# wtaylor17/ImageCFGen-Pytorch

Hardware: AMD Instinct MI355X
Metric: ALI training images/sec (E+G+D step), MorphoMNIST bs=512/GPU (higher is better)
Workload: dtype f32; 1 GPU; image_scms/mnist.py ALI iteration (EG step + 2 D steps + diagnostics), MorphoMNIST 28x28x1 synthetic, bs=512/GPU, fp32 MFMA, mode=stepper+hipgraph; global_batch=512, parallelism=dp1

## Files before the change

### imagecfgen-pytorch_amd/ali_hip/_lib.py

```python
import ctypes
import os
from ctypes import POINTER, Structure, c_char_p, c_double, c_float, c_int32, c_int64, c_size_t, c_uint64, c_void_p

_HERE = os.path.dirname(os.path.abspath(__file__))
LIB_PATH = os.path.join(_HERE, "libali_hip.so")


class AliHipUnavailable(RuntimeError):
    pass


class AliConvGeom(Structure):
    _fields_ = [(n, c_int32) for n in ("B", "H", "W", "C", "P", "Q", "K", "R", "S", "stride", "pad")]


class AliEpilogue(Structure):
    _fields_ = [("bias", c_void_p), ("act", c_int32), ("slope", c_float), ("mask", c_void_p), ("mask_ld", c_int32),
                ("dact_y", c_void_p), ("dact", c_int32), ("dslope", c_float),
                ("bn_part", c_void_p), ("bn_mode", c_int32), ("bn_groups", c_int32), ("bn_stat_mask", c_void_p),
                ("bn_mask_ld", c_int32), ("bn_x", c_void_p), ("bn_mean", c_void_p), ("bn_invstd", c_void_p),
                ("bn_mask_in", c_void_p), ("bn_mask_pre", c_void_p), ("mfma_f16", c_int32),
                ("in16", c_void_p), ("w16", c_void_p), ("out16", c_void_p),
                ("tile_order", c_void_p), ("tile_order_n", c_int32), ("in_ld", c_int32), ("out_ld", c_int32),
                ("in_ch_live", c_int32), ("bn_slots", c_int32), ("dact_y16", c_void_p)]
# ... 59 lines not shown
    "ali_act_bwd": (c_int32, [c_void_p, c_void_p, c_void_p, c_int64, c_int32, c_float, c_void_p]),
    "ali_colsum": (c_int32, [c_void_p, c_int64, c_int32, c_int32, c_void_p, c_void_p, c_size_t, c_void_p]),
    "ali_rowmask_mul": (c_int32, [c_void_p, c_void_p, c_void_p, c_int32, c_int32, c_int32, c_void_p]),
    "ali_dropout_mask": (c_int32, [c_uint64, c_uint64, c_void_p, c_float, c_void_p, c_int64, c_void_p]),
    "ali_dropout_mask_multi": (c_int32, [c_uint64, c_void_p, POINTER(c_int64), POINTER(c_float), POINTER(c_int32),
                                         POINTER(c_int32), c_int32, c_void_p, c_void_p]),
    "ali_normal_fill": (c_int32, [c_uint64, c_void_p, c_uint64, c_void_p, c_int64, c_void_p]),
    "ali_batch_gather": (c_int32, [c_void_p, c_int32, c_void_p, c_int32, c_void_p, c_void_p, c_void_p, c_int64, c_int32,
                                   c_int32, c_int32, c_int32, c_void_p, c_void_p, c_void_p, c_void_p, c_void_p]),
    "ali_bn_stats": (c_int32, [c_void_p, c_void_p, c_int32, c_int32, c_int32, c_void_p, c_void_p, c_void_p, c_void_p,
                               c_float, c_float, c_int32, c_void_p, c_void_p, c_void_p, c_void_p, c_int32, c_int64,
                               c_void_p, c_size_t, c_void_p]),
    "ali_bn_apply": (c_int32, [c_void_p, c_void_p, c_void_p, c_void_p, c_void_p, c_void_p, c_int32, c_int32, c_int32,
                               c_int32, c_int64, c_void_p]),
    "ali_bn_bwd": (c_int32, [c_void_p, c_void_p, c_void_p, c_void_p, c_void_p, c_void_p, c_void_p, c_int32, c_int32,
                             c_int32, c_int32, c_float, c_void_p, c_void_p, c_void_p, c_void_p, c_size_t, c_void_p]),
    "ali_bn_stats_from_partials": (c_int32, [c_void_p, c_int32, c_int32, c_int32, c_int64, c_void_p, c_void_p, c_void_p,
                                             c_void_p, c_float, c_float, c_void_p, c_void_p, c_void_p, c_void_p, c_int64,
                                             c_void_p]),
    "ali_bn_bwd_from_partials": (c_int32, [c_void_p, c_int32, c_void_p, c_void_p, c_void_p, c_void_p, c_void_p, c_void_p,
                                           c_void_p, c_int32, c_int32, c_int32, c_int32, c_float, c_void_p, c_void_p,
                                           c_void_p, c_void_p]),
    "ali_ew_plan": (c_int32, [c_int32, c_int64, c_int32, c_int32, c_int32, c_int32, c_int32, POINTER(c_int32)]),
    "ali_bce_logits": (c_int32, [c_void_p, c_int32, c_float, c_float, c_void_p, c_void_p, c_void_p]),
    "ali_softmax_xent": (c_int32, [c_void_p, c_void_p, c_int32, c_int32, c_float, c_void_p, c_void_p, c_void_p,
                                  c_void_p, c_void_p, c_size_t, c_void_p]),
    "ali_vae_latent_fwd": (c_int32, [c_void_p, c_void_p, c_int32, c_void_p, c_void_p, c_uint64, c_void_p, c_uint64,
                                    c_int32, c_int32, c_int32, c_float, POINTER(c_void_p), POINTER(c_int32),
                                    POINTER(c_int32), POINTER(c_void_p), c_int32, c_void_p, c_int32, c_int32, c_int32,
                                    c_void_p, c_void_p, c_void_p, c_size_t, c_void_p]),
    "ali_vae_loglik": (c_int32, [c_void_p, c_void_p, c_int32, c_int32, c_int32, c_float, c_void_p, c_float, c_float,
                                c_void_p, c_void_p, c_void_p, c_size_t, c_void_p]),
    "ali_vae_latent_bwd": (c_int32, [c_void_p, c_int32, c_void_p, c_void_p, c_void_p, c_int32, c_int32, c_int32, c_int32,
                                    c_float, c_float, c_void_p, c_void_p, c_void_p, c_int32, c_int32, c_void_p, c_void_p]),
    "ali_row_dist": (c_int32, [c_void_p, c_int32, c_void_p, c_int32, c_int64, c_int32, c_void_p, c_void_p, c_size_t,
                              c_void_p]),
    "ali_cf_hinge": (c_int32, [c_void_p, c_void_p, c_void_p, c_void_p, c_float, c_int32, c_int32, c_void_p, c_void_p,
                              c_void_p]),
    "ali_cf_join": (c_int32, [c_void_p, c_int32, c_void_p, c_void_p, c_int32, c_int32, c_int64, c_void_p, c_void_p]),
    "ali_cf_input_fwd": (c_int32, [c_void_p, c_int32, c_void_p, c_int32, POINTER(AliCfSegment), c_int32,
                                  POINTER(c_void_p), c_int32, c_int32, c_int32, c_int32, c_void_p, c_void_p, c_int32,
                                  c_void_p]),
    "ali_cf_input_step": (c_int32, [c_void_p, c_int32, c_void_p, c_void_p, c_int32, POINTER(AliCfSegment), c_int32,
                                   POINTER(c_void_p), c_int32, c_int32, c_void_p, c_void_p, c_void_p, c_int32, c_int32,
                                   c_void_p, c_double, c_double, c_double, c_double, c_void_p, c_void_p]),
    "ali_cf_select": (c_int32, [c_void_p, c_void_p, c_void_p, c_int32, c_int32, c_void_p, c_void_p, c_void_p,
# ... 138 lines not shown
```

### imagecfgen-pytorch_amd/ali_hip/chain.py

```python
import weakref
from collections import namedtuple
from typing import List, Optional

import torch
import torch.nn as nn

from . import dropout as _dropout
from . import ops
from .ops import ACT_LEAKY, ACT_NONE, ACT_TANH


def _pad4(c: int) -> int:
    return (c + 3) // 4 * 4


class Stage:
    __slots__ = ("kind", "mod", "act", "slope", "pre", "pattern", "has_drop", "drop_p", "bn", "unflat", "index", "hw")

    def __init__(self, kind, mod, pre, index):
        self.kind, self.mod, self.pre, self.index = kind, mod, pre, index
        self.act, self.slope, self.unflat = ACT_NONE, 0.0, None
        self.hw = None
        self.pattern = [k for k, _ in pre]
        self.has_drop = "drop" in self.pattern
# ... 495 lines not shown
        yield
    return (yield from gen)


def chain_forward(*args, **kwargs):
    return drive(chain_forward_gen(*args, **kwargs))


def chain_backward(*args, **kwargs):
    return drive(chain_backward_gen(*args, **kwargs))


def _pre_ops(st: Stage, sv, bn_part, mask_applied: bool, groups: int):
    cur, mask, bn = sv.x_in, sv.mask, st.bn
    B, H, W, Cp = sv.in_shape
    rows = H * W
    sv.bn_stats = None
    if bn is None:
        return ops.rowmask_mul(cur, mask, B, rows, Cp) if (mask is not None and not mask_applied) else cur
    mask_in = mask if st.pattern == ["drop", "bn"] else None
    mask_post = mask if st.pattern == ["bn", "drop"] else None
    use_batch = sv.training or bn.running_mean is None
    momentum = bn.momentum
    if bn_part is not None:
        stg = ops.bn_stats_from_partials(bn_part[0], bn_part[1], groups, Cp, (B // groups) * rows, bn.weight.detach(),
                                         bn.bias.detach(), bn.running_mean, bn.running_var, momentum, bn.eps)
    else:
        stg = ops.bn_stats(cur, mask_in, B, rows, Cp, bn.weight.detach(), bn.bias.detach(), bn.running_mean,
                           bn.running_var, momentum, bn.eps, use_batch, groups=groups)
    if use_batch and bn.num_batches_tracked is not None:
        for _ in range(groups):
            _count_batch(bn)
    sv.bn_stats = stg if groups == 1 else [stg[gi] for gi in range(groups)]
    return ops.bn_apply(cur, stg, mask_in, mask_post, B, rows, Cp, groups=groups)


def _for_next_stage(nxt: Stage, sv, groups: int, lane):
    B, P, Q, K = sv.out_shape
    draw = lambda: _dropout.next_mask(B, K, nxt.drop_p, sv.x_in.device, K, lane=lane)
    if sv.training and nxt.pattern == ["drop"] and sv.route.fold_ok:
        return draw(), None, None
    early = bn_fwd = None
    if nxt.bn is not None and sv.route.bn_leave and (sv.training or nxt.bn.running_mean is None):
        if sv.training and nxt.pattern == ["drop", "bn"]:
            early = draw()
        slots, tile_rows, pixel_major = ops.conv_mtiles(sv.geom, 0)
        rows_g = (B // groups) * (1 if pixel_major else P * Q)
        if slots > 0 and (groups == 1 or (B % groups == 0 and rows_g % tile_rows == 0
                                          and (not pixel_major or B % tile_rows == 0))):
            part = torch.empty(2 * K * slots, dtype=torch.float32, device=sv.x_in.device)
            bn_fwd = (part, groups, early, slots)
    return None, early, bn_fwd


def _launch_fwd(plan: ChainPlan, st: Stage, sv, folded, bn_fwd, out_ld: int, jmask, alloc):
    t, y, m, c_log = sv.t, sv.y, st.mod, sv.c_log
    B, H, W, Cp = sv.in_shape
# ... 178 lines not shown
        slots = ops.conv_mtiles(g, 0 if rt.dgrad == "convT" else 1)[0] if rt.bn_reduce else 0
        if slots > 0:
            bn_red = (torch.empty(2 * Cp * slots, dtype=torch.float32, device=g_pre.device), slots)
            ep = ops.epilogue(bn_bwd=(bn_red[0], sv.x_in, sv.bn_stats[0], sv.bn_stats[1], mask_in, mask_pre, slots))
        else:
            ep = ops.epilogue()
    if rt.dgrad == "tconv1" and bn is None and sv.mask is None:
        ops.tconv1_dgrad(g_pre, 1, plan.packed(st, "fwd", Cp), dact_y, pact, pslope, gt, B, H, W, Cp, m.kernel_size[0],
                         m.kernel_size[1], m.padding[0])
    elif st.kind == "convT":
        ops.conv_fwd(g, g_pre, plan.packed(st, "dgrad", Cp), gt, ep, live=(None, sv.c_log))
        yield
    else:
        wc = H * W * Cp if rt.dgrad == "flat_gemm" else Cp
        ops.conv_bwd_data(g, g_pre, plan.packed(st, "dgrad", wc), gt, ep, in_ld=ld,
                          live=(wc if rt.dgrad == "flat_gemm" else sv.c_log, None))
        yield
    if bn is None:
        return gt
    use_batch = sv.training or bn.running_mean is None
    slope = pslope if pact == ACT_LEAKY else -1.0
    out = dict(want_gx=want, out_dgamma=grad_dst.get(id(bn.weight)) if need_params else None,
               out_dbeta=grad_dst.get(id(bn.bias)) if need_params else None)
    if bn_red is not None:
        dgam, dbet, gprev = ops.bn_bwd_from_partials(bn_red[0], bn_red[1], sv.x_in, gt, mask_in, mask_pre, sv.bn_stats,
                                                     bn.weight.detach(), B, H * W, Cp, use_batch, slope, **out)
    else:
        dgam, dbet, gprev = ops.bn_bwd(sv.x_in, gt, mask_in, mask_pre, sv.bn_stats, bn.weight.detach(), B, H * W, Cp,
                                       use_batch, slope, **out)
    if need_params:
        grads[id(bn.weight)], grads[id(bn.bias)] = dgam, dbet
    if pact == ACT_TANH and gprev is not None:
        gprev = ops.act_bwd(gprev, sv.x_in, ACT_TANH, 0.0)
    return gprev


def chain_backward_gen(plan: ChainPlan, saved, gy: torch.Tensor, c_log_in: int, need_gx: bool, need_params: bool = True,
                       grad_dst=None, gx_planes=None, gy_ld: int = 0, gy_pre: bool = False, in_act=None, fold=None):
    grads = {}
    grad_dst = grad_dst or {}
    n = len(plan.stages)
    last = plan.stages[-1]
    assert saved[0].c_log == c_log_in, "chain_backward: c_log_in differs from the forward pass's"
    if gy_ld:
        if not (gy_pre or last.act == ACT_NONE) or not join_ok(plan):
            raise ValueError("chain_backward(gy_ld=...): needs join_ok(plan) and a pre-activation gradient")
        g_pre = gy
# ... 165 lines not shown
```

### imagecfgen-pytorch_amd/ali_hip/ops.py

```python
import collections
import ctypes
from ctypes import byref, c_void_p

import numpy as np
import torch

from . import _lib
from ._lib import ACT_LEAKY, ACT_NONE, ACT_TANH, AliConvGeom, AliEpilogue

_WS = {}
_WS_BYTES = 256 << 20


def set_workspace_bytes(n: int):
    global _WS_BYTES
    _WS_BYTES = int(n)
    _WS.clear()


def workspace(device, slot: int = 0) -> torch.Tensor:
    key = (device.type, device.index if device.index is not None else torch.cuda.current_device(), slot)
    ws = _WS.get(key)
    if ws is None or ws.numel() < _WS_BYTES:
        ws = torch.zeros(_WS_BYTES, dtype=torch.uint8, device=device)
# ... 813 lines not shown
    _lib.check(lib.ali_bn_stats_from_partials(_chk(part, "part"), slots, groups, C, count, _opt(gamma), _opt(beta),
                                              _opt(running_mean), _opt(running_var), momentum, eps,
                                              c_void_p(st[0, 0].data_ptr()), c_void_p(st[0, 1].data_ptr()),
                                              c_void_p(st[0, 2].data_ptr()), c_void_p(st[0, 3].data_ptr()), 4 * C,
                                              _stream()), "ali_bn_stats_from_partials")
    return st[0] if groups == 1 else st


def bn_bwd_from_partials(part, slots, x, g, mask_in, mask_pre, st, gamma, B, rows_per_img, C, batch_stats, slope,
                         want_gx=True, out_dgamma=None, out_dbeta=None):
    lib = _lib.load()
    if out_dgamma is None or out_dbeta is None:
        dg = torch.empty(2, C, dtype=torch.float32, device=x.device)
        out_dgamma, out_dbeta = dg[0], dg[1]
    gx = torch.empty_like(x) if want_gx else None
    _lib.check(lib.ali_bn_bwd_from_partials(_chk(part, "part"), slots, _chk(x, "x"), _chk(g, "g"), _opt(mask_in),
                                            _opt(mask_pre), c_void_p(st[0].data_ptr()), c_void_p(st[1].data_ptr()),
                                            _opt(gamma), B, rows_per_img, C, int(batch_stats), float(slope),
                                            _chk(out_dgamma, "dgamma"), _chk(out_dbeta, "dbeta"), _opt(gx), _stream()),
               "ali_bn_bwd_from_partials")
    return out_dgamma, out_dbeta, gx


def bn_apply(x, st, mask_in, mask_post, B, rows_per_img, C, out=None, groups=1):
    lib = _lib.load()
    out = torch.empty_like(x) if out is None else out
    st0 = st if groups == 1 else st[0]
    _lib.check(lib.ali_bn_apply(_chk(x, "x"), c_void_p(st0[2].data_ptr()), c_void_p(st0[3].data_ptr()), _opt(mask_in),
                                _opt(mask_post), _chk(out), B, rows_per_img, C, groups, 4 * C, _stream()),
               "ali_bn_apply")
    return out


def bn_bwd(x, g, mask_in, mask_pre, st, gamma, B, rows_per_img, C, batch_stats, slope, want_gx=True, out_dgamma=None,
           out_dbeta=None):
    lib = _lib.load()
    ws = workspace(x.device)
    if out_dgamma is None or out_dbeta is None:
        dg = torch.empty(2, C, dtype=torch.float32, device=x.device)
        out_dgamma, out_dbeta = dg[0], dg[1]
    gx = torch.empty_like(x) if want_gx else None
    _lib.check(lib.ali_bn_bwd(_chk(x, "x"), _chk(g, "g"), _opt(mask_in), _opt(mask_pre), c_void_p(st[0].data_ptr()),
                              c_void_p(st[1].data_ptr()), _opt(gamma), B, rows_per_img, C, int(batch_stats),
                              float(slope), _chk(out_dgamma, "dgamma"), _chk(out_dbeta, "dbeta"), _opt(gx),
                              c_void_p(ws.data_ptr()), ws.numel(), _stream()), "ali_bn_bwd")
    return out_dgamma, out_dbeta, gx
# ... 1181 lines not shown
```

### imagecfgen-pytorch_amd/csrc/elementwise.hip

```cpp
#include "ali_common.h"
#include <algorithm>
#include <string.h>

namespace ali {

constexpr int kEwBlock = 256;
static inline int ew_grid(long long n, int per_thread = 1) {
  long long b = (n + (long long)kEwBlock * per_thread - 1) / ((long long)kEwBlock * per_thread);
  if (b > 2048) b = 2048;
  if (b < 1) b = 1;
  return (int)b;
}

__global__ void pack_weights_kernel(const float* __restrict__ src, float* __restrict__ dst, int N, int T, int C,
                                    int Cpad, long long s_n, long long s_tap, long long s_c) {
  const long long total = (long long)N * T * Cpad;
  long long i = (long long)blockIdx.x * blockDim.x + threadIdx.x;
  const long long step = (long long)gridDim.x * blockDim.x;
  for (; i < total; i += step) {
    const int c = (int)(i % Cpad);
    const long long nt = i / Cpad;
    const int tp = (int)(nt % T);
    const long long n = nt / T;
    dst[i] = c < C ? src[n * s_n + tp * s_tap + c * s_c] : 0.f;
// ... 214 lines not shown
  red2[t] = s2;
  __syncthreads();
  for (int off = lanes_r / 2; off > 0; off >>= 1) {
    if (tr < off) {
      red1[t] += red1[t + off * lanes_c];
      red2[t] += red2[t + off * lanes_c];
    }
    __syncthreads();
  }
  if (tr == 0 && tc < C) {
    part[((long long)blockIdx.x * 2 + 0) * C + tc] = red1[t];
    part[((long long)blockIdx.x * 2 + 1) * C + tc] = red2[t];
  }
}
struct PartLayout { long long g, b, s, c; };
__device__ __forceinline__ double block_sum_256(double v, double* red) {
  v = wave_sum(v);
  if ((threadIdx.x & 63) == 0) red[threadIdx.x >> 6] = v;
  __syncthreads();
  const double tot = ((red[0] + red[1]) + red[2]) + red[3];
  __syncthreads();
  return tot;
}
__global__ void __launch_bounds__(kEwBlock)
bn_stats_final_kernel(const float* __restrict__ part, PartLayout lay, int nblk, int C, long long count,
                      const float* __restrict__ gamma, const float* __restrict__ beta,
                      float* __restrict__ running_mean, float* __restrict__ running_var, float momentum, float eps,
                      int training, float* __restrict__ mean_out, float* __restrict__ invstd_out, float* __restrict__ sc,
                      float* __restrict__ sh, int groups, long long stat_stride) {
  __shared__ double red[8];
  const int c = blockIdx.x;
  for (int gi = 0; gi < groups; ++gi) {
    const float* pg = part + (long long)gi * lay.g + (long long)c * lay.c;
    float mean, var;
    if (training) {
      double s1 = 0.0, s2 = 0.0;
      for (int b = threadIdx.x; b < nblk; b += kEwBlock) {
        s1 += (double)pg[(long long)b * lay.b];
        s2 += (double)pg[(long long)b * lay.b + lay.s];
      }
      s1 = block_sum_256(s1, red);
      s2 = block_sum_256(s2, red + 4);
      const double m = s1 / (double)count;
      double v = s2 / (double)count - m * m;
      if (v < 0.0) v = 0.0;
      mean = (float)m;
      var = (float)v;
      if (running_mean && threadIdx.x == 0) {
        const double unb = count > 1 ? v * (double)count / (double)(count - 1) : v;
        running_mean[c] = (1.f - momentum) * running_mean[c] + momentum * mean;
        running_var[c] = (1.f - momentum) * running_var[c] + momentum * (float)unb;
      }
    } else {
      mean = running_mean[c];
      var = running_var[c];
    }
    if (threadIdx.x == 0) {
      const float invstd = 1.f / sqrtf(var + eps);
      const float g = gamma ? gamma[c] : 1.f, b = beta ? beta[c] : 0.f;
      const long long o = (long long)gi * stat_stride + c;
      mean_out[o] = mean;
      invstd_out[o] = invstd;
      sc[o] = g * invstd;
      sh[o] = b - mean * g * invstd;
    }
  }
}
__global__ void bn_apply_kernel(const float* __restrict__ x, const float* __restrict__ sc, const float* __restrict__ sh,
                                const float* __restrict__ mask_in, const float* __restrict__ mask_post,
                                float* __restrict__ out, long long n, int rows_per_img, int C) {
  long long i = (long long)blockIdx.x * blockDim.x + threadIdx.x;
  const long long step = (long long)gridDim.x * blockDim.x;
  const long long per_img = (long long)rows_per_img * C;
  for (; i < n; i += step) {
    const int c = (int)(i % C);
    const long long img = i / per_img;
    float v = x[i];
    if (mask_in) v *= mask_in[img * C + c];
    v = v * sc[c] + sh[c];
    if (mask_post) v *= mask_post[img * C + c];
    out[i] = v;
  }
}
__global__ void bn_bwd_partial_kernel(const float* __restrict__ x, const float* __restrict__ g,
                                      const float* __restrict__ mask_in, const float* __restrict__ mask_pre,
                                      const float* __restrict__ mean, const float* __restrict__ invstd,
                                      long long rows, int rows_per_img, int C, float* __restrict__ part) {
// ... 209 lines not shown
  for (unsigned r = blockIdx.x * lanes_r + tr; r < rows; r += stride) {
    const float4 xr = ld4(x + (size_t)r * C + c);
    float4 gv = ld4(g + (size_t)r * C + c);
    const unsigned img = (mask_in || mask_pre) ? r / rows_per_img : 0u;
    const float4 mi = mask_in ? ld4(mask_in + (size_t)img * C + c) : one;
    if (mask_pre) gv = mul4(gv, ld4(mask_pre + (size_t)img * C + c));
    const float4 xv = mul4(xr, mi);
    float4 o = gv;
    if (batch_stats) {
      o.x -= (db.x + (xv.x - mu.x) * is.x * dg.x) * inv_count;
      o.y -= (db.y + (xv.y - mu.y) * is.y * dg.y) * inv_count;
      o.z -= (db.z + (xv.z - mu.z) * is.z * dg.z) * inv_count;
      o.w -= (db.w + (xv.w - mu.w) * is.w * dg.w) * inv_count;
    }
    o = mul4(mul4(o, k), mi);
    if (slope >= 0.f) {
      o.x *= xr.x > 0.f ? 1.f : slope; o.y *= xr.y > 0.f ? 1.f : slope;
      o.z *= xr.z > 0.f ? 1.f : slope; o.w *= xr.w > 0.f ? 1.f : slope;
    }
    *reinterpret_cast<float4*>(gx + (size_t)r * C + c) = o;
  }
}

static bool vec_ok(long long rows, int C) {
  return (C % 4) == 0 && C >= 4 && C <= 4 * kEwBlock && rows * C < (1LL << 31);
}
static int reduce_blocks_vec(long long rows, int C) {
  const int lanes_r = kEwBlock / (C / 4);
  long long nb = (rows + (long long)lanes_r * 8 - 1) / ((long long)lanes_r * 8);
  if (nb > 512) nb = 512;
  if (nb < 1) nb = 1;
  return (int)nb;
}
static int reduce_blocks(long long rows, int C) {
  int lanes_c = 1;
  const int cw = C < kEwBlock ? C : kEwBlock;
  while (lanes_c < cw) lanes_c <<= 1;
  const int lanes_r = kEwBlock / lanes_c;
  long long nb = (rows + (long long)lanes_r * 8 - 1) / ((long long)lanes_r * 8);
  if (nb > 512) nb = 512;
  if (nb < 1) nb = 1;
  return (int)nb;
}

struct EwPlan {
  bool vec;
// ... 10 lines not shown
  if ((op == ALI_EW_OP_BN_STATS || op == ALI_EW_OP_BN_BWD) && C > kEwBlock) {
    set_error("ali_ew_plan: C must be <= 256 for the reduction passes of ali_bn_stats / ali_bn_bwd");
    return ALI_ERR_BAD_ARG;
  }
  if (op == ALI_EW_OP_COLSUM && ld < C) { set_error("ali_ew_plan: ld < C"); return ALI_ERR_BAD_ARG; }
  const long long n = rows * C;
  if (op == ALI_EW_OP_ACT_BWD) { pl.ew = ew_grid(n); return ALI_OK; }
  pl.vec = vec_ok(rows * groups, C) && aligned;
  if (op == ALI_EW_OP_COLSUM) pl.vec = pl.vec && (ld % 4) == 0 && rows * ld < (1LL << 31);
  if (op == ALI_EW_OP_BN_STATS || op == ALI_EW_OP_BN_BWD || op == ALI_EW_OP_COLSUM)
    pl.nb = pl.vec ? reduce_blocks_vec(rows, C) : reduce_blocks(rows, C);
  if (op == ALI_EW_OP_BN_APPLY || op == ALI_EW_OP_BN_BWD || op == ALI_EW_OP_BN_BWD_FROM_PARTIALS)
    pl.ew = pl.vec ? ew_grid(n / 4) : ew_grid(n);
  return ALI_OK;
}

extern "C" int32_t ali_ew_plan(int32_t op, int64_t rows_per_group, int32_t rows_per_img, int32_t C, int32_t ld,
                               int32_t groups, int32_t aligned, int32_t* out_blocks) {
  EwPlan pl;
  const int rc = ew_plan(op, rows_per_group, rows_per_img, C, ld, groups, aligned != 0, pl);
  if (rc) return rc;
  if (out_blocks) { out_blocks[0] = pl.nb; out_blocks[1] = pl.ew; }
  return pl.vec ? 1 : 0;
}

constexpr int kPtgMaxChunks = 8;
__global__ void __launch_bounds__(256)
plane_table_grad_kernel(const float* __restrict__ g, int g_ld, int g_ch, const float* __restrict__ x, int x_ld, int x_ch,
                        const int* __restrict__ idx, int idx_ld, int idx_col, int B, int H, int W, int n_rows,
                        float* __restrict__ out, const float* __restrict__ table) {
  __shared__ float red[64][4];
  const int cell = blockIdx.x, ch = cell >> 4, cw = cell & 15, t = threadIdx.x, wave = t >> 6;
  const int h0 = (ch * H + 15) / 16, h1 = ((ch + 1) * H + 15) / 16;
  const int w0 = (cw * W + 15) / 16, w1 = ((cw + 1) * W + 15) / 16;
  float val[kPtgMaxChunks];
  int cls[kPtgMaxChunks];
#pragma unroll
  for (int c = 0; c < kPtgMaxChunks; ++c) {
    const int b = c * 256 + t;
    val[c] = 0.f;
    cls[c] = -1;
    if (b < B) {
      cls[c] = idx[(long long)b * idx_ld + idx_col];
      const float pt = table ? tanhf(table[cls[c] * 256 + cell]) : 0.f;
      float acc = 0.f;
      for (int h = h0; h < h1; ++h)
// ... 773 lines not shown

extern "C" int ali_bn_bwd_from_partials(const float* part, int32_t slots, const float* x, const float* g,
                                        const float* mask_in, const float* mask_pre, const float* mean,
                                        const float* invstd, const float* gamma, int32_t B, int32_t rows_per_img,
                                        int32_t C, int32_t batch_stats, float lrelu_slope, float* dgamma, float* dbeta,
                                        float* gx, ali_stream_t stream) {
  if (!part || slots <= 0 || !x || !g || !mean || !invstd || !dgamma || !dbeta || B <= 0 || rows_per_img <= 0 || C <= 0) {
    set_error("ali_bn_bwd_from_partials: bad argument");
    return ALI_ERR_BAD_ARG;
  }
  const long long rows = (long long)B * rows_per_img;
  const bool aligned = aligned16(x) && aligned16(g) && (!gx || aligned16(gx)) && (!mask_in || aligned16(mask_in)) &&
                       (!mask_pre || aligned16(mask_pre)) && aligned16(mean) && aligned16(invstd);
  EwPlan pl;
  const int rc = ew_plan(ALI_EW_OP_BN_BWD_FROM_PARTIALS, rows, rows_per_img, C, C, 1, aligned, pl);
  if (rc) return rc;
  const PartLayout lay = {0LL, 1LL, (long long)C * slots, (long long)slots};
  hipLaunchKernelGGL(bn_bwd_final_kernel, dim3(C), dim3(kEwBlock), 0, ST(stream), part, lay, slots, C, dgamma, dbeta);
  if (gx) launch_bn_bwd_apply(x, g, mask_in, mask_pre, mean, invstd, gamma, dgamma, dbeta, rows, rows_per_img, C,
                              batch_stats, lrelu_slope, gx, pl, ST(stream));
  return check_launch("bn_bwd_from_partials");
}

extern "C" int ali_plane_table_grad(const float* g, int32_t g_ld, int32_t g_ch, const float* x, int32_t x_ld, int32_t x_ch,
                                    const int32_t* idx, int32_t idx_ld, int32_t idx_col, int32_t B, int32_t H, int32_t W,
                                    int32_t n_rows, float* out, const float* table, ali_stream_t stream) {
  if (!g || (!x && !table) || !idx || !out || B <= 0 || B > 256 * kPtgMaxChunks || H <= 0 || W <= 0 || n_rows <= 0 || g_ch < 0 ||
      g_ch >= g_ld || (x && (x_ch < 0 || x_ch >= x_ld)) || idx_col < 0 || idx_col >= idx_ld) {
    set_error("ali_plane_table_grad: bad argument (B <= 2048)");
    return ALI_ERR_BAD_ARG;
  }
  hipLaunchKernelGGL(plane_table_grad_kernel, dim3(256), dim3(256), 0, ST(stream), g, g_ld, g_ch, x, x_ld, x_ch, idx, idx_ld,
                     idx_col, B, H, W, n_rows, out, table);
  return check_launch("plane_table_grad_kernel");
}

extern "C" int ali_col2im(const float* contrib, int32_t ldc, const float* bias, float* out, int32_t B, int32_t H,
                          int32_t W, int32_t Hout, int32_t Wout, int32_t NC, int32_t ostride, int32_t R, int32_t S,
                          int32_t stride, int32_t pad, int32_t act, float slope, ali_stream_t stream) {
  if (!contrib || !out || B <= 0 || H <= 0 || W <= 0 || Hout <= 0 || Wout <= 0 || NC < 1 || NC > 8 || ostride < NC ||
      R <= 0 || S <= 0 || stride <= 0 || pad < 0 || ldc < NC * R * S) {
    set_error("ali_col2im: bad argument");
    return ALI_ERR_BAD_ARG;
  }
  const long long total = (long long)B * Hout * Wout;
  const dim3 grid(ew_grid(total)), block(kEwBlock);
// ... 139 lines not shown
```

### include/ali_hip.h

```cpp
#ifndef ALI_HIP_H
#define ALI_HIP_H

#include <stddef.h>
#include <stdint.h>

#ifdef __cplusplus
extern "C" {
#endif

typedef void* ali_stream_t;
#define ALI_WS_RESERVED 4096

typedef enum {
  ALI_OK = 0,
  ALI_ERR_BAD_ARG = -1,
  ALI_ERR_WORKSPACE = -2,
  ALI_ERR_LAUNCH = -3
} AliStatus;

typedef enum { ALI_ACT_NONE = 0, ALI_ACT_LEAKY = 1, ALI_ACT_TANH = 2 } AliAct;

typedef struct {
  int32_t B, H, W, C;
  int32_t P, Q, K;
// ... 150 lines not shown
                 float* out, int32_t B, int32_t rows_per_img, int32_t C, int32_t groups, int64_t stat_stride,
                 ali_stream_t stream);
int ali_bn_bwd(const float* x, const float* g, const float* mask_in, const float* mask_pre,
               const float* mean, const float* invstd, const float* gamma,
               int32_t B, int32_t rows_per_img, int32_t C, int32_t batch_stats, float lrelu_slope,
               float* dgamma, float* dbeta, float* gx, void* ws, size_t ws_bytes, ali_stream_t stream);

int ali_bn_stats_from_partials(const float* part, int32_t slots, int32_t groups, int32_t C, int64_t count,
                               const float* gamma, const float* beta, float* running_mean, float* running_var,
                               float momentum, float eps, float* mean, float* invstd, float* sc, float* sh,
                               int64_t stat_stride, ali_stream_t stream);
int ali_bn_bwd_from_partials(const float* part, int32_t slots, const float* x, const float* g, const float* mask_in,
                             const float* mask_pre, const float* mean, const float* invstd, const float* gamma,
                             int32_t B, int32_t rows_per_img, int32_t C, int32_t batch_stats, float lrelu_slope,
                             float* dgamma, float* dbeta, float* gx, ali_stream_t stream);
#define ALI_EW_OP_BN_STATS 0
#define ALI_EW_OP_BN_APPLY 1
#define ALI_EW_OP_BN_BWD 2
#define ALI_EW_OP_BN_BWD_FROM_PARTIALS 3
#define ALI_EW_OP_COLSUM 4
#define ALI_EW_OP_ACT_BWD 5
int32_t ali_ew_plan(int32_t op, int64_t rows_per_group, int32_t rows_per_img, int32_t C, int32_t ld, int32_t groups,
                    int32_t aligned, int32_t* out_blocks);

int ali_bce_logits(const float* logit, int32_t B, float target, float gscale, float* out2, float* glogit,
                   ali_stream_t stream);

int ali_softmax_xent(const float* logit, const float* target, int32_t B, int32_t C, float gscale, float* out2,
                     float* glogit, int32_t* pred, int64_t* hits_accum, void* ws, size_t ws_bytes, ali_stream_t stream);

int ali_vae_latent_fwd(const float* mean, const float* log_var, int32_t head_ld, const float* eps, float* eps_out,
                       uint64_t seed, const int64_t* dev_counter, uint64_t offset, int32_t S, int32_t B, int32_t L,
                       float k, const void* const* onehot, const int32_t* n_classes, const int32_t* onehot_is_int,
                       const float* const* tables, int32_t n_emb, const float* cont, int32_t n_cont, int32_t write_cond,
                       int32_t ld, float* out, float* kl_out, void* ws, size_t ws_bytes, ali_stream_t stream);
int ali_vae_loglik(const float* x, const float* xhat, int32_t B, int32_t S, int32_t P, float log_var,
                   const float* kl_sum, float kl_weight, float gscale, float* out3, float* gxhat, void* ws,
                   size_t ws_bytes, ali_stream_t stream);
int ali_vae_latent_bwd(const float* gin, int32_t ld, const float* eps, const float* mean, const float* log_var,
                       int32_t head_ld, int32_t S, int32_t B, int32_t L, float k, float kl_weight, const float* kl_scale,
                       float* gmean, float* glog_var, int32_t gld, int32_t ncond, float* gcond, ali_stream_t stream);

#define ALI_DIST_L1 0
#define ALI_DIST_L2 1
#define ALI_CF_COPY 0
#define ALI_CF_TANH 1
// ... 214 lines not shown
```

Measured before the change: 84960 images/s.

## Fold BN partial-stat reduction into apply and backward-apply kernels

Adds fused kernels that reduce the per-block BatchNorm partial sums inside each apply block, then normalize the activations in the same launch. This applies to the forward pass and to the backward input-gradient pass. It replaces a separate finalize kernel plus an apply kernel, removing one launch and one round trip of the statistics per BN layer. In exchange, every block redundantly re-reads the partial-sum slab. A planner gates the fused path by shape, slab size and re-read ratio, and falls back to the old path otherwise.

```diff
diff --git a/imagecfgen-pytorch_amd/ali_hip/_lib.py b/imagecfgen-pytorch_amd/ali_hip/_lib.py
--- a/imagecfgen-pytorch_amd/ali_hip/_lib.py
+++ b/imagecfgen-pytorch_amd/ali_hip/_lib.py
@@ -105,6 +105,14 @@
                                            c_void_p, c_int32, c_int32, c_int32, c_int32, c_float, c_void_p, c_void_p,
                                            c_void_p, c_void_p]),
     "ali_ew_plan": (c_int32, [c_int32, c_int64, c_int32, c_int32, c_int32, c_int32, c_int32, POINTER(c_int32)]),
+    "ali_bn_apply_from_partials": (c_int32, [c_void_p, c_int32, c_int32, c_int32, c_void_p, c_void_p, c_void_p,
+                                             c_void_p, c_float, c_float, c_void_p, c_void_p, c_void_p, c_void_p, c_int64,
+                                             c_void_p, c_void_p, c_void_p, c_void_p, c_int32, c_int32, c_int32, c_int32,
+                                             c_void_p]),
+    "ali_bn_bwd_apply_from_partials": (c_int32, [c_void_p, c_int32, c_void_p, c_void_p, c_void_p, c_void_p, c_void_p,
+                                                 c_void_p, c_void_p, c_int32, c_int32, c_int32, c_int32, c_float,
+                                                 c_void_p, c_void_p, c_void_p, c_int32, c_int32, c_void_p]),
+    "ali_bn_fold_plan": (c_int32, [c_int32, c_int64, c_int32, c_int32, c_int32, c_int32, POINTER(c_int32)]),
     "ali_bce_logits": (c_int32, [c_void_p, c_int32, c_float, c_float, c_void_p, c_void_p, c_void_p]),
     "ali_softmax_xent": (c_int32, [c_void_p, c_void_p, c_int32, c_int32, c_float, c_void_p, c_void_p, c_void_p,
                                   c_void_p, c_void_p, c_size_t, c_void_p]),
diff --git a/imagecfgen-pytorch_amd/ali_hip/chain.py b/imagecfgen-pytorch_amd/ali_hip/chain.py
--- a/imagecfgen-pytorch_amd/ali_hip/chain.py
+++ b/imagecfgen-pytorch_amd/ali_hip/chain.py
@@ -541,7 +541,12 @@
     mask_post = mask if st.pattern == ["bn", "drop"] else None
     use_batch = sv.training or bn.running_mean is None
     momentum = bn.momentum
-    if bn_part is not None:
+    out = None
+    if bn_part is not None and ops.bn_fold_fwd_ok(bn_part[0], bn_part[1], groups, Cp, cur, mask_in, mask_post, B, rows):
+        stg, out = ops.bn_apply_from_partials(bn_part[0], bn_part[1], groups, Cp, bn.weight.detach(), bn.bias.detach(),
+                                              bn.running_mean, bn.running_var, momentum, bn.eps, cur, mask_in,
+                                              mask_post, B, rows)
+    elif bn_part is not None:
         stg = ops.bn_stats_from_partials(bn_part[0], bn_part[1], groups, Cp, (B // groups) * rows, bn.weight.detach(),
                                          bn.bias.detach(), bn.running_mean, bn.running_var, momentum, bn.eps)
     else:
@@ -551,7 +556,7 @@
         for _ in range(groups):
             _count_batch(bn)
     sv.bn_stats = stg if groups == 1 else [stg[gi] for gi in range(groups)]
-    return ops.bn_apply(cur, stg, mask_in, mask_post, B, rows, Cp, groups=groups)
+    return out if out is not None else ops.bn_apply(cur, stg, mask_in, mask_post, B, rows, Cp, groups=groups)
 
 
 def _for_next_stage(nxt: Stage, sv, groups: int, lane):
@@ -776,7 +781,13 @@
     slope = pslope if pact == ACT_LEAKY else -1.0
     out = dict(want_gx=want, out_dgamma=grad_dst.get(id(bn.weight)) if need_params else None,
                out_dbeta=grad_dst.get(id(bn.bias)) if need_params else None)
-    if bn_red is not None:
+    if bn_red is not None and ops.bn_fold_bwd_ok(bn_red[1], sv.x_in, gt, mask_in, mask_pre, sv.bn_stats, B, H * W, Cp,
+                                                 want):
+        dgam, dbet, gprev = ops.bn_bwd_apply_from_partials(bn_red[0], bn_red[1], sv.x_in, gt, mask_in, mask_pre,
+                                                           sv.bn_stats, bn.weight.detach(), B, H * W, Cp, use_batch,
+                                                           slope, out_dgamma=out["out_dgamma"],
+                                                           out_dbeta=out["out_dbeta"])
+    elif bn_red is not None:
         dgam, dbet, gprev = ops.bn_bwd_from_partials(bn_red[0], bn_red[1], sv.x_in, gt, mask_in, mask_pre, sv.bn_stats,
                                                      bn.weight.detach(), B, H * W, Cp, use_batch, slope, **out)
     else:
diff --git a/imagecfgen-pytorch_amd/ali_hip/ops.py b/imagecfgen-pytorch_amd/ali_hip/ops.py
--- a/imagecfgen-pytorch_amd/ali_hip/ops.py
+++ b/imagecfgen-pytorch_amd/ali_hip/ops.py
@@ -859,6 +859,66 @@
     return out_dgamma, out_dbeta, gx
 
 
+BN_FOLD = __import__("os").environ.get("ALI_NO_BN_FOLD", "0") in ("", "0")
+BN_FOLD_TAKEN = {"fwd": 0, "bwd": 0}
+
+
+def bn_fold_plan(direction, rows_per_group, C, slots_per_group, groups=1, aligned=True):
+    out = (ctypes.c_int32 * 2)(0, 0)
+    code = _lib.load().ali_bn_fold_plan({"fwd": 0, "bwd": 1}[direction], rows_per_group, C, slots_per_group, groups,
+                                        int(bool(aligned)), out)
+    _lib.check(min(code, 0), "ali_bn_fold_plan")
+    return (out[0], out[1]) if code == 1 else None
+
+
+def _aligned(*ts):
+    return all(t is None or t.data_ptr() % 16 == 0 for t in ts)
+
+
+def bn_fold_fwd_ok(part, slots, groups, C, x, mask_in, mask_post, B, rows_per_img):
+    return BN_FOLD and bn_fold_plan("fwd", (B // groups) * rows_per_img, C, slots // groups, groups,
+                                    _aligned(x, mask_in, mask_post)) is not None
+
+
+def bn_fold_bwd_ok(slots, x, g, mask_in, mask_pre, st, B, rows_per_img, C, want_gx):
+    return want_gx and BN_FOLD and bn_fold_plan("bwd", B * rows_per_img, C, slots, 1,
+                                                _aligned(x, g, mask_in, mask_pre, st[0], st[1])) is not None
+
+
+def bn_apply_from_partials(part, slots, groups, C, gamma, beta, running_mean, running_var, momentum, eps, x, mask_in,
+                           mask_post, B, rows_per_img, out=None, force=None):
+    lib = _lib.load()
+    st = torch.empty(groups, 4, C, dtype=torch.float32, device=part.device)
+    out = torch.empty_like(x) if out is None else out
+    slab, chunks = force or (0, 0)
+    _lib.check(lib.ali_bn_apply_from_partials(_chk(part, "part"), slots, groups, C, _opt(gamma), _opt(beta),
+                                              _opt(running_mean), _opt(running_var), momentum, eps,
+                                              c_void_p(st[0, 0].data_ptr()), c_void_p(st[0, 1].data_ptr()),
+                                              c_void_p(st[0, 2].data_ptr()), c_void_p(st[0, 3].data_ptr()), 4 * C,
+                                              _chk(x, "x"), _opt(mask_in), _opt(mask_post), _chk(out, "out"), B,
+                                              rows_per_img, slab, chunks, _stream()), "ali_bn_apply_from_partials")
+    BN_FOLD_TAKEN["fwd"] += 1
+    return (st[0] if groups == 1 else st), out
+
+
+def bn_bwd_apply_from_partials(part, slots, x, g, mask_in, mask_pre, st, gamma, B, rows_per_img, C, batch_stats, slope,
+                               out_dgamma=None, out_dbeta=None, force=None):
+    lib = _lib.load()
+    if out_dgamma is None or out_dbeta is None:
+        dg = torch.empty(2, C, dtype=torch.float32, device=x.device)
+        out_dgamma, out_dbeta = dg[0], dg[1]
+    gx = torch.empty_like(x)
+    slab, chunks = force or (0, 0)
+    _lib.check(lib.ali_bn_bwd_apply_from_partials(_chk(part, "part"), slots, _chk(x, "x"), _chk(g, "g"), _opt(mask_in),
+                                                  _opt(mask_pre), c_void_p(st[0].data_ptr()),
+                                                  c_void_p(st[1].data_ptr()), _opt(gamma), B, rows_per_img, C,
+                                                  int(batch_stats), float(slope), _chk(out_dgamma, "dgamma"),
+                                                  _chk(out_dbeta, "dbeta"), _chk(gx, "gx"), slab, chunks, _stream()),
+               "ali_bn_bwd_apply_from_partials")
+    BN_FOLD_TAKEN["bwd"] += 1
+    return out_dgamma, out_dbeta, gx
+
+
 def bn_apply(x, st, mask_in, mask_post, B, rows_per_img, C, out=None, groups=1):
     lib = _lib.load()
     out = torch.empty_like(x) if out is None else out
diff --git a/imagecfgen-pytorch_amd/csrc/elementwise.hip b/imagecfgen-pytorch_amd/csrc/elementwise.hip
--- a/imagecfgen-pytorch_amd/csrc/elementwise.hip
+++ b/imagecfgen-pytorch_amd/csrc/elementwise.hip
@@ -260,6 +260,28 @@
   __syncthreads();
   return tot;
 }
+__device__ __forceinline__ void bn_batch_moments(double s1, double s2, long long count, float& mean, float& var,
+                                                 double& vd) {
+  const double m = s1 / (double)count;
+  double v = s2 / (double)count - m * m;
+  if (v < 0.0) v = 0.0;
+  mean = (float)m;
+  var = (float)v;
+  vd = v;
+}
+__device__ __forceinline__ void bn_running_update(float* __restrict__ running_mean, float* __restrict__ running_var,
+                                                  int c, float mean, double v, long long count, float momentum) {
+  const double unb = count > 1 ? v * (double)count / (double)(count - 1) : v;
+  running_mean[c] = (1.f - momentum) * running_mean[c] + momentum * mean;
+  running_var[c] = (1.f - momentum) * running_var[c] + momentum * (float)unb;
+}
+__device__ __forceinline__ void bn_affine(float mean, float var, float eps, const float* __restrict__ gamma,
+                                          const float* __restrict__ beta, int c, float& invstd, float& sc, float& sh) {
+  invstd = 1.f / sqrtf(var + eps);
+  const float g = gamma ? gamma[c] : 1.f, b = beta ? beta[c] : 0.f;
+  sc = g * invstd;
+  sh = b - mean * g * invstd;
+}
 __global__ void __launch_bounds__(kEwBlock)
 bn_stats_final_kernel(const float* __restrict__ part, PartLayout lay, int nblk, int C, long long count,
                       const float* __restrict__ gamma, const float* __restrict__ beta,
@@ -279,28 +301,21 @@
       }
       s1 = block_sum_256(s1, red);
       s2 = block_sum_256(s2, red + 4);
-      const double m = s1 / (double)count;
-      double v = s2 / (double)count - m * m;
-      if (v < 0.0) v = 0.0;
-      mean = (float)m;
-      var = (float)v;
-      if (running_mean && threadIdx.x == 0) {
-        const double unb = count > 1 ? v * (double)count / (double)(count - 1) : v;
-        running_mean[c] = (1.f - momentum) * running_mean[c] + momentum * mean;
-        running_var[c] = (1.f - momentum) * running_var[c] + momentum * (float)unb;
-      }
+      double v;
+      bn_batch_moments(s1, s2, count, mean, var, v);
+      if (running_mean && threadIdx.x == 0) bn_running_update(running_mean, running_var, c, mean, v, count, momentum);
     } else {
       mean = running_mean[c];
       var = running_var[c];
     }
     if (threadIdx.x == 0) {
-      const float invstd = 1.f / sqrtf(var + eps);
-      const float g = gamma ? gamma[c] : 1.f, b = beta ? beta[c] : 0.f;
+      float invstd, a, b;
+      bn_affine(mean, var, eps, gamma, beta, c, invstd, a, b);
       const long long o = (long long)gi * stat_stride + c;
       mean_out[o] = mean;
       invstd_out[o] = invstd;
-      sc[o] = g * invstd;
-      sh[o] = b - mean * g * invstd;
+      sc[o] = a;
+      sh[o] = b;
     }
   }
 }
@@ -556,6 +571,149 @@
   }
 }
 
+struct FoldGrid { int nchunk, nslab, W; };
+__device__ __forceinline__ void fold_block(const FoldGrid& fg, int& chunk, int& slab) {
+  const int run = fg.W * fg.nslab, q = blockIdx.x / run, r = blockIdx.x - q * run;
+  slab = r / fg.W;
+  chunk = q * fg.W + (r - slab * fg.W);
+}
+template <int S>
+__device__ __forceinline__ void slab_sums(const float* __restrict__ p, long long cs, long long ss, int per,
+                                          double (*red)[4]) {
+  double a1[S], a2[S];
+#pragma unroll
+  for (int j = 0; j < S; ++j) a1[j] = a2[j] = 0.0;
+  for (int b = threadIdx.x; b < per; b += kEwBlock) {
+#pragma unroll
+    for (int j = 0; j < S; ++j) {
+      a1[j] += (double)p[j * cs + b];
+      a2[j] += (double)p[ss + j * cs + b];
+    }
+  }
+  const int w = threadIdx.x >> 6;
+  const bool lead = (threadIdx.x & 63) == 0;
+#pragma unroll
+  for (int j = 0; j < S; ++j) {
+    const double v1 = wave_sum(a1[j]), v2 = wave_sum(a2[j]);
+    if (lead) {
+      red[j][w] = v1;
+      red[S + j][w] = v2;
+    }
+  }
+  __syncthreads();
+}
+__device__ __forceinline__ double red_total(const double* r) { return ((r[0] + r[1]) + r[2]) + r[3]; }
+
+template <int S>
+__global__ void __launch_bounds__(kEwBlock)
+bn_fold_apply_kernel(const float* __restrict__ part, int slots, int per, FoldGrid fg, long long count,
+                     const float* __restrict__ gamma, const float* __restrict__ beta, float* __restrict__ running_mean,
+                     float* __restrict__ running_var, float momentum, float eps, float* __restrict__ mean_out,
+                     float* __restrict__ invstd_out, float* __restrict__ sc_out, float* __restrict__ sh_out,
+                     long long stat_stride, int groups, const float* __restrict__ x, const float* __restrict__ mask_in,
+                     const float* __restrict__ mask_post, float* __restrict__ out, unsigned rows,
+                     unsigned rows_per_img, unsigned C) {
+  __shared__ double red[2 * S][4];
+  int chunk, slab;
+  fold_block(fg, chunk, slab);
+  const int gi = blockIdx.y;
+  constexpr unsigned C4 = S / 4, lanes_r = kEwBlock / C4;
+  const unsigned tr = threadIdx.x / C4, jc = (threadIdx.x - tr * C4) * 4, c = slab * S + jc;
+  const long long cs = slots, ss = (long long)C * slots;
+  const bool lead = chunk == 0 && gi == 0;
+  const int g0 = lead ? 0 : gi, g1 = lead ? groups : gi + 1;
+  float sca[4], shb[4];
+  for (int g = g0; g < g1; ++g) {
+    if (g != g0) __syncthreads();
+    slab_sums<S>(part + (long long)g * per + (long long)slab * S * slots, cs, ss, per, red);
+#pragma unroll
+    for (int k = 0; k < 4; ++k) {
+      float mean, var, invstd, a, b;
+      double v;
+      bn_batch_moments(red_total(red[jc + k]), red_total(red[S + jc + k]), count, mean, var, v);
+      bn_affine(mean, var, eps, gamma, beta, c + k, invstd, a, b);
+      if (g == gi) {
+        sca[k] = a;
+        shb[k] = b;
+      }
+      if (lead && tr == 0) {
+        if (running_mean) bn_running_update(running_mean, running_var, c + k, mean, v, count, momentum);
+        const long long o = (long long)g * stat_stride + c + k;
+        mean_out[o] = mean;
+        invstd_out[o] = invstd;
+        sc_out[o] = a;
+        sh_out[o] = b;
+      }
+    }
+  }
+  x += (size_t)gi * rows * C;
+  out += (size_t)gi * rows * C;
+  if (mask_in) mask_in += (size_t)gi * (rows / rows_per_img) * C;
+  if (mask_post) mask_post += (size_t)gi * (rows / rows_per_img) * C;
+  const float4 a = make_float4(sca[0], sca[1], sca[2], sca[3]), b = make_float4(shb[0], shb[1], shb[2], shb[3]);
+  const unsigned stride = fg.nchunk * lanes_r;
+  for (unsigned r = chunk * lanes_r + tr; r < rows; r += stride) {
+    float4 v = ld4(x + (size_t)r * C + c);
+    const unsigned img = (mask_in || mask_post) ? r / rows_per_img : 0u;
+    if (mask_in) v = mul4(v, ld4(mask_in + (size_t)img * C + c));
+    v.x = v.x * a.x + b.x; v.y = v.y * a.y + b.y; v.z = v.z * a.z + b.z; v.w = v.w * a.w + b.w;
+    if (mask_post) v = mul4(v, ld4(mask_post + (size_t)img * C + c));
+    *reinterpret_cast<float4*>(out + (size_t)r * C + c) = v;
+  }
+}
+
+template <int S>
+__global__ void __launch_bounds__(kEwBlock)
+bn_fold_bwd_apply_kernel(const float* __restrict__ part, int slots, FoldGrid fg, const float* __restrict__ x,
+                         const float* __restrict__ g, const float* __restrict__ mask_in,
+                         const float* __restrict__ mask_pre, const float* __restrict__ mean,
+                         const float* __restrict__ invstd, const float* __restrict__ gamma, float* __restrict__ dgamma,
+                         float* __restrict__ dbeta, unsigned rows, unsigned rows_per_img, unsigned C, float inv_count,
+                         int batch_stats, float slope, float* __restrict__ gx) {
+  __shared__ double red[2 * S][4];
+  int chunk, slab;
+  fold_block(fg, chunk, slab);
+  constexpr unsigned C4 = S / 4, lanes_r = kEwBlock / C4;
+  const unsigned tr = threadIdx.x / C4, jc = (threadIdx.x - tr * C4) * 4, c = slab * S + jc;
+  slab_sums<S>(part + (long long)slab * S * slots, slots, (long long)C * slots, slots, red);
+  float dgs[4], dbs[4];
+#pragma unroll
+  for (int k = 0; k < 4; ++k) {
+    dgs[k] = (float)red_total(red[jc + k]);
+    dbs[k] = (float)red_total(red[S + jc + k]);
+    if (chunk == 0 && tr == 0) {
+      dgamma[c + k] = dgs[k];
+      dbeta[c + k] = dbs[k];
+    }
+  }
+  const float4 one = make_float4(1.f, 1.f, 1.f, 1.f);
+  const float4 is = ldc4(invstd + c), mu = ldc4(mean + c), gm = gamma ? ldc4(gamma + c) : one;
+  const float4 dg = make_float4(dgs[0], dgs[1], dgs[2], dgs[3]), db = make_float4(dbs[0], dbs[1], dbs[2], dbs[3]);
+  const float4 k = mul4(gm, is);
+  const unsigned stride = fg.nchunk * lanes_r;
+  for (unsigned r = chunk * lanes_r + tr; r < rows; r += stride) {
+    const float4 xr = ld4(x + (size_t)r * C + c);
+    float4 gv = ld4(g + (size_t)r * C + c);
+    const unsigned img = (mask_in || mask_pre) ? r / rows_per_img : 0u;
+    const float4 mi = mask_in ? ld4(mask_in + (size_t)img * C + c) : one;
+    if (mask_pre) gv = mul4(gv, ld4(mask_pre + (size_t)img * C + c));
+    const float4 xv = mul4(xr, mi);
+    float4 o = gv;
+    if (batch_stats) {
+      o.x -= (db.x + (xv.x - mu.x) * is.x * dg.x) * inv_count;
+      o.y -= (db.y + (xv.y - mu.y) * is.y * dg.y) * inv_count;
+      o.z -= (db.z + (xv.z - mu.z) * is.z * dg.z) * inv_count;
+      o.w -= (db.w + (xv.w - mu.w) * is.w * dg.w) * inv_count;
+    }
+    o = mul4(mul4(o, k), mi);
+    if (slope >= 0.f) {
+      o.x *= xr.x > 0.f ? 1.f : slope; o.y *= xr.y > 0.f ? 1.f : slope;
+      o.z *= xr.z > 0.f ? 1.f : slope; o.w *= xr.w > 0.f ? 1.f : slope;
+    }
+    *reinterpret_cast<float4*>(gx + (size_t)r * C + c) = o;
+  }
+}
+
 static bool vec_ok(long long rows, int C) {
   return (C % 4) == 0 && C >= 4 && C <= 4 * kEwBlock && rows * C < (1LL << 31);
 }
@@ -612,6 +770,49 @@
   if (rc) return rc;
   if (out_blocks) { out_blocks[0] = pl.nb; out_blocks[1] = pl.ew; }
   return pl.vec ? 1 : 0;
+}
+
+constexpr int kFoldSlabFloats = 16384;
+constexpr int kFoldReread = 4;
+constexpr int kFoldBlocks = 512;
+struct FoldPlan { int S, nchunk; };
+static bool fold_shape_ok(long long rows, int C, int groups, bool aligned) {
+  return aligned && vec_ok(rows * groups, C);
+}
+static int fold_w(int nchunk) { return nchunk < 8 ? nchunk : 8; }
+static int fold_plan(int dir, long long rows, int C, int per, int groups, bool aligned, FoldPlan& fp) {
+  fp = FoldPlan{0, 0};
+  if ((dir != 0 && dir != 1) || rows <= 0 || C <= 0 || per <= 0 || groups < 1 || (dir == 1 && groups != 1)) {
+    set_error("ali_bn_fold_plan: bad argument");
+    return ALI_ERR_BAD_ARG;
+  }
+  if (!fold_shape_ok(rows, C, groups, aligned)) return ALI_OK;
+  int S = 0;
+  for (int s = 16; s >= 4 && !S; s >>= 1)
+    if (C % s == 0 && 2LL * s * per <= kFoldSlabFloats) S = s;
+  if (!S) return ALI_OK;
+  const int nslab = C / S;
+  const long long lanes_r = kEwBlock / (S / 4);
+  const long long passes = (rows + lanes_r - 1) / lanes_r;
+  const long long part_bytes = 2LL * C * per * 4, row_bytes = rows * C * 4 * (dir == 0 ? 1 : 2);
+  long long nc = std::min<long long>(kFoldBlocks / ((long long)nslab * groups), passes);
+  nc = std::min<long long>(nc, row_bytes / (kFoldReread * part_bytes));
+  if (nc > 8) nc -= nc % 8;
+  if (nc < 1) return ALI_OK;
+  fp = FoldPlan{S, (int)nc};
+  return ALI_OK;
+}
+static bool fold_forced_ok(int S, int nchunk, int C) {
+  return (S == 4 || S == 8 || S == 16 || S == 32) && C % S == 0 && nchunk >= 1 && nchunk % fold_w(nchunk) == 0;
+}
+
+extern "C" int32_t ali_bn_fold_plan(int32_t dir, int64_t rows_per_group, int32_t C, int32_t slots_per_group,
+                                    int32_t groups, int32_t aligned, int32_t* out) {
+  FoldPlan fp;
+  const int rc = fold_plan(dir, rows_per_group, C, slots_per_group, groups, aligned != 0, fp);
+  if (rc) return rc;
+  if (out) { out[0] = fp.S; out[1] = fp.nchunk; }
+  return fp.S ? 1 : 0;
 }
 
 constexpr int kPtgMaxChunks = 8;
@@ -1431,6 +1632,94 @@
   return check_launch("bn_bwd_from_partials");
 }
 
+static int fold_resolve(const char* who, int dir, long long rows, int C, int per, int groups, bool aligned, int slab,
+                        int chunks, FoldPlan& fp) {
+  if (slab > 0 || chunks > 0) {
+    if (!fold_shape_ok(rows, C, groups, aligned) || !fold_forced_ok(slab, chunks, C)) {
+      set_error("%s: forced slab %d x %d chunks does not fit the shape (C %% 4, alignment, < 2^31 elements)", who, slab,
+                chunks);
+      return ALI_ERR_BAD_ARG;
+    }
+    fp = FoldPlan{slab, chunks};
+    return ALI_OK;
+  }
+  const int rc = fold_plan(dir, rows, C, per, groups, aligned, fp);
+  if (rc) return rc;
+  if (!fp.S) {
+    set_error("%s: the fold plan refuses this shape (ali_bn_fold_plan)", who);
+    return ALI_ERR_BAD_ARG;
+  }
+  return ALI_OK;
+}
+
+extern "C" int ali_bn_apply_from_partials(const float* part, int32_t slots, int32_t groups, int32_t C,
+                                          const float* gamma, const float* beta, float* running_mean,
+                                          float* running_var, float momentum, float eps, float* mean, float* invstd,
+                                          float* sc, float* sh, int64_t stat_stride, const float* x,
+                                          const float* mask_in, const float* mask_post, float* out, int32_t B,
+                                          int32_t rows_per_img, int32_t slab, int32_t chunks, ali_stream_t stream) {
+  if (!part || slots <= 0 || groups < 1 || slots % groups != 0 || C <= 0 || !mean || !invstd || !sc || !sh ||
+      (groups > 1 && stat_stride < C) || !x || !out || B <= 0 || rows_per_img <= 0 || B % groups != 0 ||
+      (!running_mean) != (!running_var)) {
+    set_error("ali_bn_apply_from_partials: bad argument");
+    return ALI_ERR_BAD_ARG;
+  }
+  const int per = slots / groups;
+  const long long rows = (long long)(B / groups) * rows_per_img;
+  const bool aligned = aligned16(x) && aligned16(out) && (!mask_in || aligned16(mask_in)) &&
+                       (!mask_post || aligned16(mask_post));
+  FoldPlan fp;
+  const int rc = fold_resolve("ali_bn_apply_from_partials", 0, rows, C, per, groups, aligned, slab, chunks, fp);
+  if (rc) return rc;
+  const FoldGrid fg = {fp.nchunk, C / fp.S, fold_w(fp.nchunk)};
+  const dim3 grid(fp.nchunk * fg.nslab, groups);
+#define ALI_FOLD_FWD(SW)                                                                                               \
+  hipLaunchKernelGGL(bn_fold_apply_kernel<SW>, grid, dim3(kEwBlock), 0, ST(stream), part, slots, per, fg, rows, gamma,   \
+                     beta, running_mean, running_var, momentum, eps, mean, invstd, sc, sh, (long long)stat_stride,     \
+                     groups, x, mask_in, mask_post, out, (unsigned)rows, (unsigned)rows_per_img, (unsigned)C)
+  switch (fp.S) {
+    case 4: ALI_FOLD_FWD(4); break;
+    case 8: ALI_FOLD_FWD(8); break;
+    case 16: ALI_FOLD_FWD(16); break;
+    default: ALI_FOLD_FWD(32); break;
+  }
+#undef ALI_FOLD_FWD
+  return check_launch("bn_fold_apply_kernel");
+}
+
+extern "C" int ali_bn_bwd_apply_from_partials(const float* part, int32_t slots, const float* x, const float* g,
+                                              const float* mask_in, const float* mask_pre, const float* mean,
+                                              const float* invstd, const float* gamma, int32_t B,
+                                              int32_t rows_per_img, int32_t C, int32_t batch_stats, float lrelu_slope,
+                                              float* dgamma, float* dbeta, float* gx, int32_t slab, int32_t chunks,
+                                              ali_stream_t stream) {
+  if (!part || slots <= 0 || !x || !g || !mean || !invstd || !dgamma || !dbeta || !gx || B <= 0 || rows_per_img <= 0 ||
+      C <= 0) {
+    set_error("ali_bn_bwd_apply_from_partials: bad argument");
+    return ALI_ERR_BAD_ARG;
+  }
+  const long long rows = (long long)B * rows_per_img;
+  const bool aligned = aligned16(x) && aligned16(g) && aligned16(gx) && (!mask_in || aligned16(mask_in)) &&
+                       (!mask_pre || aligned16(mask_pre)) && aligned16(mean) && aligned16(invstd);
+  FoldPlan fp;
+  const int rc = fold_resolve("ali_bn_bwd_apply_from_partials", 1, rows, C, slots, 1, aligned, slab, chunks, fp);
+  if (rc) return rc;
+  const FoldGrid fg = {fp.nchunk, C / fp.S, fold_w(fp.nchunk)};
+  const dim3 grid(fp.nchunk * fg.nslab);
+#define ALI_FOLD_BWD(SW)                                                                                               \
+  hipLaunchKernelGGL(bn_fold_bwd_apply_kernel<SW>, grid, dim3(kEwBlock), 0, ST(stream), part, slots, fg, x, g, mask_in, \
+                     mask_pre, mean, invstd, gamma, dgamma, dbeta, (unsigned)rows, (unsigned)rows_per_img,             \
+                     (unsigned)C, 1.f / (float)rows, batch_stats, lrelu_slope, gx)
+  switch (fp.S) {
+    case 4: ALI_FOLD_BWD(4); break;
+    case 8: ALI_FOLD_BWD(8); break;
+    case 16: ALI_FOLD_BWD(16); break;
+    default: ALI_FOLD_BWD(32); break;
+  }
+#undef ALI_FOLD_BWD
+  return check_launch("bn_fold_bwd_apply_kernel");
+}
+
 extern "C" int ali_plane_table_grad(const float* g, int32_t g_ld, int32_t g_ch, const float* x, int32_t x_ld, int32_t x_ch,
                                     const int32_t* idx, int32_t idx_ld, int32_t idx_col, int32_t B, int32_t H, int32_t W,
                                     int32_t n_rows, float* out, const float* table, ali_stream_t stream) {
diff --git a/include/ali_hip.h b/include/ali_hip.h
--- a/include/ali_hip.h
+++ b/include/ali_hip.h
@@ -196,6 +196,18 @@
 #define ALI_EW_OP_ACT_BWD 5
 int32_t ali_ew_plan(int32_t op, int64_t rows_per_group, int32_t rows_per_img, int32_t C, int32_t ld, int32_t groups,
                     int32_t aligned, int32_t* out_blocks);
+int ali_bn_apply_from_partials(const float* part, int32_t slots, int32_t groups, int32_t C, const float* gamma,
+                               const float* beta, float* running_mean, float* running_var, float momentum, float eps,
+                               float* mean, float* invstd, float* sc, float* sh, int64_t stat_stride, const float* x,
+                               const float* mask_in, const float* mask_post, float* out, int32_t B,
+                               int32_t rows_per_img, int32_t slab, int32_t chunks, ali_stream_t stream);
+int ali_bn_bwd_apply_from_partials(const float* part, int32_t slots, const float* x, const float* g,
+                                   const float* mask_in, const float* mask_pre, const float* mean, const float* invstd,
+                                   const float* gamma, int32_t B, int32_t rows_per_img, int32_t C, int32_t batch_stats,
+                                   float lrelu_slope, float* dgamma, float* dbeta, float* gx, int32_t slab,
+                                   int32_t chunks, ali_stream_t stream);
+int32_t ali_bn_fold_plan(int32_t dir, int64_t rows_per_group, int32_t C, int32_t slots_per_group, int32_t groups,
+                         int32_t aligned, int32_t* out);
 
 int ali_bce_logits(const float* logit, int32_t B, float target, float gscale, float* out2, float* glogit,
                    ali_stream_t stream);
```

New measurement: 76060 images/s. -10.5%, worse.
